# victorramirez952/tomography_3d_reconstructor

Measured on AMD Instinct MI355X. Metric: Mvoxels/s (SDF+MC) on 1024^3 ellipsoid stack; achieved HBM GB/s vs peak, higher is better.
Workload: dtype f64

## Files before the change

include/tomo_hip.h:

```cpp
#ifndef TOMO_HIP_H
#define TOMO_HIP_H

#include <stddef.h>
#include <stdint.h>

#ifdef __cplusplus
extern "C" {
#endif

#define TOMO_OK 0
#define TOMO_E_ARG (-1)
#define TOMO_E_LAUNCH (-2)
#define TOMO_E_SIZE (-3)
#define TOMO_E_WORKSPACE (-4)

int tomo_abi_version(void);
const char *tomo_error_string(int code);
int tomo_host_mc_cell(const float *h_v, double iso, int8_t *h_tris, int *h_uses_centre);
double tomo_host_mc_edge_offset(double va, double vb);
void tomo_host_mc_centre_offset(const double *h_v8, double *h_out3);

int tomo_host_checksum(const void *h_data, int64_t nbytes, int nthreads, uint64_t *h_out);
int tomo_host_checksum_impl(const void *h_data, int64_t nbytes, int nthreads, int impl, uint64_t *h_out);
int64_t tomo_host_checksum_chunk_bytes(void);
// ... 208 lines not shown
                        unsigned long long *vox_key, int64_t cap, void *stream);
int tomo_mc_eval_capped(const float *field, int Nz, int Ny, int Nx, int64_t pitch, int xorg, double iso,
                        const unsigned long long *vox_key, int64_t cap, const unsigned long long *na_dev,
                        uint32_t *vox_counts, uint8_t *vox_flags, void *stream);
int tomo_mc_emit(const float *field, int Nz, int Ny, int Nx, int64_t pitch, int xorg, double iso,
                 const unsigned long long *vox_key, int64_t na, const unsigned long long *seg_act,
                 const uint32_t *seg_aoff, const uint32_t *vox_voff, const uint32_t *vox_foff, const uint8_t *vox_flags,
                 int z_offset, unsigned long long *vkey, float *vpos, int32_t *faces, unsigned long long *totals,
                 void *stream);

int tomo_mc_first_touch(const float *field, int Nz, int Ny, int Nx, int64_t pitch, int xorg, double iso,
                        const unsigned long long *vox_key, int64_t na, const unsigned long long *seg_act,
                        const uint32_t *seg_aoff, const uint32_t *vox_voff, const uint8_t *vox_flags, int mode,
                        uint32_t *created, const uint32_t *base, int32_t *ft_rank, unsigned long long *totals, void *stream);

int tomo_mc3_list(int Nz, int Ny, int Nx, int xorg, const uint32_t *seg_cnt, const unsigned long long *seg_act,
                  uint32_t *seg_blk, uint32_t *seg_aoff, unsigned long long *vox_key, int64_t cap, unsigned long long *tot,
                  void *stream);
int tomo_mc3_eval(const float *field, int Nz, int Ny, int Nx, int64_t pitch, int xorg, double iso,
                  const unsigned long long *vox_key, int64_t cap, const unsigned long long *tot, int z_offset,
                  uint32_t *vox_loc, int32_t *vox_til, uint8_t *vox_flags, uint16_t *vox_used, float *vox_f3, float *vox_c3,
                  uint32_t *blk3, void *stream);
int64_t tomo_mc3_slice_table_words(int Nz, int Ny);
int64_t tomo_mc3_sort_segments(int Nz, int Ny);
int tomo_mc3_scan(int Nz, int Ny, int Nx, int xorg, const uint32_t *seg_aoff, const uint32_t *vox_loc, int64_t cap,
                  uint32_t *blk3, uint32_t *slice_tab, unsigned long long *tot, int64_t cap_v, int64_t cap_f, void *stream);
int tomo_mc3_vertices(int Nz, int Ny, int Nx, int xorg, const unsigned long long *vox_key, int64_t cap,
                      const unsigned long long *tot, const uint32_t *vox_loc, const uint8_t *vox_flags, const float *vox_f3,
                      const float *vox_c3, const uint32_t *blk3, const uint32_t *slice_tab, int z_offset, int shift,
                      const double *cum, int64_t ncum, const double *adj, int64_t nadj, float mm_y, float mm_x, float *vrec,
                      uint32_t *keys, uint32_t *idx, void *stream);
int64_t tomo_mc3_sort_workspace_bytes(int64_t cap_v, int64_t nseg);
int tomo_mc3_sort_rank_top(const float *vrec, uint32_t *keys, uint32_t *idx, int64_t cap_v, int Nz, int Ny, const uint32_t *slice_tab,
                           unsigned long long *tot, float *uniq, int32_t *table, void *workspace, int64_t workspace_bytes,
                           float z_top, void *stream);
int tomo_mc3_sort_rank_fused(const float *vrec, const uint32_t *keys, int64_t cap_v, int Nz, int Ny, uint32_t *slice_tab,
                             unsigned long long *tot, float *uniq, int32_t *table, float z_top, void *stream);
int tomo_mc3_faces(int Nz, int Ny, int Nx, int xorg, const unsigned long long *vox_key, int64_t cap, unsigned long long *tot,
                   const unsigned long long *seg_act, const uint32_t *seg_aoff, const uint32_t *vox_loc, const int32_t *vox_til,
                   const uint16_t *vox_used, const uint32_t *blk3, const int32_t *table, int64_t *faces, int64_t cap_f,
                   void *stream);
// ... 48 lines not shown
```

tomography_3d_reconstructor_amd/_lib.py:

```python
import ctypes
import os
import subprocess

_HERE = os.path.dirname(os.path.abspath(__file__))
SO_PATH = os.environ.get("TOMO_LIB") or os.path.join(_HERE, "libtomo_hip.so")
CSRC = os.path.join(_HERE, "csrc")

_c_i = ctypes.c_int
_c_i64 = ctypes.c_int64
_c_p = ctypes.c_void_p
_c_d = ctypes.c_double
_c_f = ctypes.c_float

SIGNATURES = {
    "tomo_abi_version": (_c_i, []),
    "tomo_error_string": (ctypes.c_char_p, [_c_i]),
    "tomo_host_mc_cell": (_c_i, [_c_p, _c_d, _c_p, _c_p]),
    "tomo_host_mc_edge_offset": (_c_d, [_c_d, _c_d]),
    "tomo_host_mc_centre_offset": (None, [_c_p, _c_p]),
    "tomo_host_checksum": (_c_i, [_c_p, _c_i64, _c_i, _c_p]),
    "tomo_host_checksum_impl": (_c_i, [_c_p, _c_i64, _c_i, _c_i, _c_p]),
    "tomo_host_checksum_chunk_bytes": (_c_i64, []),
    "tomo_host_checksum_part": (_c_i, [_c_p, _c_i64, _c_i64, _c_i, _c_i, _c_p]),
    "tomo_host_checksum_fold": (_c_i, [_c_p, _c_i64, _c_i64, _c_p]),
# ... 111 lines not shown
    "tomo_sign_rows": (_c_i64, [_c_i]),
    "tomo_sign_buffer_words": (_c_i64, [_c_i, _c_i, _c_i, _c_i]),
    "tomo_field_signs": (_c_i, [_c_p, _c_i, _c_i, _c_i, _c_i64, _c_i, _c_d, _c_i, _c_i, _c_p, _c_p, _c_p]),
    "tomo_mc_classify": (_c_i, [_c_p, _c_p, _c_i, _c_i, _c_i, _c_i, _c_p, _c_p, _c_p]),
    "tomo_mc_scan_segments": (_c_i, [_c_p, _c_i64, _c_p, _c_p, _c_p, _c_i64, _c_p]),
    "tomo_mc_scan_workspace_bytes": (_c_i64, [_c_i64]),
    "tomo_mc_scan": (_c_i, [_c_p, _c_i64, _c_p, _c_p, _c_p, _c_p, _c_i64, _c_p]),
    "tomo_mc_list": (_c_i, [_c_i, _c_i, _c_i, _c_i, _c_p, _c_p, _c_p, _c_p]),
    "tomo_mc_eval": (_c_i, [_c_p, _c_i, _c_i, _c_i, _c_i64, _c_i, _c_d, _c_p, _c_i64, _c_p, _c_p, _c_p]),
    "tomo_mc_list_capped": (_c_i, [_c_i, _c_i, _c_i, _c_i, _c_p, _c_p, _c_p, _c_i64, _c_p]),
    "tomo_mc_eval_capped": (_c_i, [_c_p, _c_i, _c_i, _c_i, _c_i64, _c_i, _c_d, _c_p, _c_i64, _c_p, _c_p, _c_p, _c_p]),
    "tomo_mc_emit": (_c_i, [_c_p, _c_i, _c_i, _c_i, _c_i64, _c_i, _c_d, _c_p, _c_i64, _c_p, _c_p, _c_p, _c_p, _c_p, _c_i, _c_p,
                            _c_p, _c_p, _c_p, _c_p]),
    "tomo_mc_first_touch": (_c_i, [_c_p, _c_i, _c_i, _c_i, _c_i64, _c_i, _c_d, _c_p, _c_i64, _c_p, _c_p, _c_p, _c_p, _c_i, _c_p,
                                   _c_p, _c_p, _c_p, _c_p]),
    "tomo_mc3_list": (_c_i, [_c_i, _c_i, _c_i, _c_i, _c_p, _c_p, _c_p, _c_p, _c_p, _c_i64, _c_p, _c_p]),
    "tomo_mc3_eval": (_c_i, [_c_p, _c_i, _c_i, _c_i, _c_i64, _c_i, _c_d, _c_p, _c_i64, _c_p, _c_i, _c_p, _c_p, _c_p, _c_p, _c_p,
                             _c_p, _c_p, _c_p]),
    "tomo_mc3_slice_table_words": (_c_i64, [_c_i, _c_i]),
    "tomo_mc3_sort_segments": (_c_i64, [_c_i, _c_i]),
    "tomo_mc3_scan": (_c_i, [_c_i, _c_i, _c_i, _c_i, _c_p, _c_p, _c_i64, _c_p, _c_p, _c_p, _c_i64, _c_i64, _c_p]),
    "tomo_mc3_vertices": (_c_i, [_c_i, _c_i, _c_i, _c_i, _c_p, _c_i64, _c_p, _c_p, _c_p, _c_p, _c_p, _c_p, _c_p, _c_i, _c_i,
                                 _c_p, _c_i64, _c_p, _c_i64, _c_f, _c_f, _c_p, _c_p, _c_p, _c_p]),
    "tomo_mc3_sort_workspace_bytes": (_c_i64, [_c_i64, _c_i64]),
    "tomo_mc3_sort_rank_top": (_c_i, [_c_p, _c_p, _c_p, _c_i64, _c_i, _c_i, _c_p, _c_p, _c_p, _c_p, _c_p, _c_i64, _c_f, _c_p]),
    "tomo_mc3_sort_rank_fused": (_c_i, [_c_p, _c_p, _c_i64, _c_i, _c_i, _c_p, _c_p, _c_p, _c_p, _c_f, _c_p]),
    "tomo_mc3_faces": (_c_i, [_c_i, _c_i, _c_i, _c_i, _c_p, _c_i64, _c_p, _c_p, _c_p, _c_p, _c_p, _c_p, _c_p, _c_p, _c_p, _c_i64, _c_p]),
    "tomo_vertex_finalize": (_c_i, [_c_p, _c_i64, _c_i, _c_p, _c_i64, _c_p, _c_i64, _c_f, _c_f, _c_p]),
    "tomo_mesh_unique_workspace_bytes": (_c_i64, [_c_i64]),
    "tomo_mesh_unique": (_c_i, [_c_p, _c_i64, _c_p, _c_p, _c_p, _c_p, _c_i64, _c_p]),
    "tomo_mesh_lookup": (_c_i, [_c_p, _c_i64, _c_p, _c_i64, _c_p, _c_p, _c_p]),
    "tomo_slab_top_rows": (_c_i, [_c_p, _c_p, _c_i64, _c_i64, _c_p, _c_p]),
    "tomo_slab_lookup_summary": (_c_i, [_c_p, _c_p, _c_i64, _c_p, _c_i64, _c_p, _c_i64, _c_i64, _c_p, _c_p, _c_p]),
    "tomo_mc3_faces_slab": (_c_i, [_c_i, _c_i, _c_i, _c_i, _c_p, _c_i64, _c_p, _c_p, _c_p, _c_p, _c_p, _c_p, _c_p, _c_p, _c_p, _c_i64,
                                   _c_p, _c_i, _c_i, _c_p, _c_i64, _c_i64, _c_p]),
    "tomo_mesh_volume_area": (_c_i, [_c_p, _c_p, _c_i64, _c_p, _c_p]),
# ... 60 lines not shown
```

tomography_3d_reconstructor_amd/csrc/mc.hip:

```cpp
#include <cstring>
#include <cstdlib>
#include "tomo_common.h"
#include <rocprim/rocprim.hpp>

#define MC_LUT_QUAL __device__ const
#define MC_FN __device__ static inline
#include "mc_cell.h"

#define SEG 256
#define KEY_XBITS 20
static_assert(KEY_XBITS + 2 == TOMO_KEY_ROW_SHIFT, "key layout shared with mesh.hip");

struct McGrid {
    int Nz, Ny, Nx;
    int64_t pitch;
    int xorg;
    int segs_per_row;
    double iso;
};

typedef float float4u __attribute__((ext_vector_type(4), aligned(4)));
typedef float float2u __attribute__((ext_vector_type(2), aligned(4)));
typedef float float3u __attribute__((ext_vector_type(3), aligned(4)));
typedef int int3u __attribute__((ext_vector_type(3), aligned(4)));
// ... 692 lines not shown
        return TOMO_E_ARG;
    if (na <= 0) return TOMO_OK;
    int64_t blocks = ceil_div64(na, 256);
    if (blocks > 0x7fffffff) return TOMO_E_SIZE;
    hipLaunchKernelGGL(mc_first_touch_kernel, dim3((unsigned)blocks), dim3(256), 0, (hipStream_t)stream, field, g,
                       (const u64 *)vox_key, na, (const u64 *)seg_act, seg_aoff, vox_voff, vox_flags, mode, created, base, ft_rank,
                       (u64 *)totals);
    return tomo_status();
}

#define MC3_BLK 256
#define MC3_LOC_A(l) ((l) & 1023u)
#define MC3_LOC_B(l) (((l) >> 10) & 1023u)
#define MC3_LOC_T(l) ((l) >> 20)

__global__ __launch_bounds__(256) void mc3_segsum_kernel(const u32 *__restrict__ seg_cnt, int64_t nseg, u32 *__restrict__ seg_blk,
                                                         int64_t nblk)
{
    const int lane = threadIdx.x & 63;
    const int64_t b = (int64_t)blockIdx.x * 4 + (threadIdx.x >> 6);
    if (b >= nblk) return;
    const int64_t i0 = b * MC3_BLK + lane * 4;
    u32 s = 0;
    if (i0 + 3 < nseg) {
        const uint4 v = *(const uint4 *)(seg_cnt + i0);
        s = v.x + v.y + v.z + v.w;
    } else {
        for (int k = 0; k < 4; k++) if (i0 + k < nseg) s += seg_cnt[i0 + k];
    }
    s = wave_sum(s);
    if (lane == 0) seg_blk[b] = s;
}

template <int K>
__device__ static inline void scan_small_inplace(u32 *__restrict__ a, int64_t stride, int64_t n, u64 *total_out, u32 *lds )
{
    const int lane = threadIdx.x & 63, w = threadIdx.x >> 6;
    u32 carry[K];
    u64 wide[K];
#pragma unroll
    for (int k = 0; k < K; k++) { carry[k] = 0; wide[k] = 0; }
    for (int64_t base = 0; base < n; base += 1024 * 8) {
        const int64_t i0 = base + (int64_t)threadIdx.x * 8;
        u32 v[K][8], s[K];
#pragma unroll
        for (int k = 0; k < K; k++) {
            u32 *p = a + k * stride + i0;
            if (i0 + 7 < n && ((uintptr_t)p & 15) == 0) {
                const uint4 lo = *(const uint4 *)p, hi = *(const uint4 *)(p + 4);
                v[k][0] = lo.x; v[k][1] = lo.y; v[k][2] = lo.z; v[k][3] = lo.w; v[k][4] = hi.x; v[k][5] = hi.y; v[k][6] = hi.z; v[k][7] = hi.w;
            } else {
#pragma unroll
                for (int j = 0; j < 8; j++) v[k][j] = i0 + j < n ? p[j] : 0u;
            }
            s[k] = 0;
#pragma unroll
            for (int j = 0; j < 8; j++) s[k] += v[k][j];
        }
        u32 inc[K];
#pragma unroll
        for (int k = 0; k < K; k++) {
            inc[k] = wave_inclusive_scan(s[k]);
            if (lane == 63) lds[k * 16 + w] = inc[k];
        }
        __syncthreads();
        if (w == 0) {
#pragma unroll
            for (int k = 0; k < K; k++) {
                const u32 t = lane < 16 ? lds[k * 16 + lane] : 0u;
                const u32 ti = wave_inclusive_scan(t);
                if (lane < 16) lds[k * 16 + lane] = ti - t;
                if (lane == 15) lds[K * 16 + k] = ti;
            }
        }
        __syncthreads();
#pragma unroll
        for (int k = 0; k < K; k++) {
            u32 ex = carry[k] + lds[k * 16 + w] + inc[k] - s[k];
            u32 *p = a + k * stride + i0;
            if (i0 + 7 < n && ((uintptr_t)p & 15) == 0) {
                uint4 lo, hi;
                lo.x = ex; ex += v[k][0]; lo.y = ex; ex += v[k][1]; lo.z = ex; ex += v[k][2]; lo.w = ex; ex += v[k][3];
                hi.x = ex; ex += v[k][4]; hi.y = ex; ex += v[k][5]; hi.z = ex; ex += v[k][6]; hi.w = ex;
                *(uint4 *)p = lo; *(uint4 *)(p + 4) = hi;
            } else {
#pragma unroll
                for (int j = 0; j < 8; j++) { if (i0 + j < n) p[j] = ex; ex += v[k][j]; }
            }
            carry[k] += lds[K * 16 + k];
            wide[k] += lds[K * 16 + k];
        }
        __syncthreads();
    }
#pragma unroll
    for (int k = 0; k < K; k++) total_out[k] = wide[k];
}

__global__ __launch_bounds__(1024) void mc3_scan_seg_kernel(u32 *__restrict__ seg_blk, int64_t nblk, u64 *__restrict__ tot)
{
    __shared__ u32 lds[17];
    u64 total;
    scan_small_inplace<1>(seg_blk, 0, nblk, &total, lds);
    if (threadIdx.x == 0) {
        tot[0] = total;
        tot[1] = tot[2] = tot[4] = tot[5] = tot[6] = tot[7] = 0ull;
        tot[3] = total > 0xffffffffull ? 1ull : 0ull;
    }
}

__global__ __launch_bounds__(MC3_BLK) void mc3_list_kernel(const McGrid g, const u32 *__restrict__ seg_cnt,
                                                           const u32 *__restrict__ seg_blk, const u64 *__restrict__ seg_act,
                                                           int64_t nseg, u32 *__restrict__ seg_aoff, u64 *__restrict__ vox_key,
                                                           u32 cap, u64 *__restrict__ tot)
{
    __shared__ u32 wsum[4];
    const int lane = threadIdx.x & 63, w = threadIdx.x >> 6;
    const int64_t seg = (int64_t)blockIdx.x * MC3_BLK + threadIdx.x;
    const u32 cnt = seg < nseg ? seg_cnt[seg] : 0u;
// ... 1 lines not shown
    if (lane == 63) wsum[w] = inc;
    __syncthreads();
    u32 o = seg_blk[blockIdx.x] + inc - cnt;
    for (int k = 0; k < w; k++) o += wsum[k];
    if (seg >= nseg) return;
    seg_aoff[seg] = o;
    if (seg == nseg - 1) seg_aoff[nseg] = o + cnt;
    if (cnt == 0) return;
    if ((u64)o + cnt > (u64)cap || tot[0] > (u64)cap) {
        if (o <= cap) atomicOr((unsigned long long *)&tot[3], 1ull);
        return;
    }
    seg_write_keys(g, seg, seg_act, o, vox_key);
}

TOMO_API int tomo_mc3_list(int Nz, int Ny, int Nx, int xorg, const uint32_t *seg_cnt, const unsigned long long *seg_act,
                           uint32_t *seg_blk, uint32_t *seg_aoff, unsigned long long *vox_key, int64_t cap,
                           unsigned long long *tot, void *stream)
{
    if (!seg_cnt || !seg_act || !seg_blk || !seg_aoff || !vox_key || !tot) return TOMO_E_ARG;
    McGrid g;
    if (const int rc = index_grid(g, Nz, Ny, Nx, xorg)) return rc;
    if (cap <= 0 || cap >= 0x1fffffffll) return TOMO_E_SIZE;
    const int64_t nseg = (int64_t)Nz * Ny * g.segs_per_row, nblk = ceil_div64(nseg, MC3_BLK);
    if (nblk > 0x7fffffff) return TOMO_E_SIZE;
    hipStream_t s = (hipStream_t)stream;
    hipLaunchKernelGGL(mc3_segsum_kernel, dim3((unsigned)ceil_div64(nblk, 4)), dim3(256), 0, s, seg_cnt, nseg, seg_blk, nblk);
    hipLaunchKernelGGL(mc3_scan_seg_kernel, dim3(1), dim3(1024), 0, s, seg_blk, nblk, (u64 *)tot);
    hipLaunchKernelGGL(mc3_list_kernel, dim3((unsigned)nblk), dim3(MC3_BLK), 0, s, g, seg_cnt, (const u32 *)seg_blk,
                       (const u64 *)seg_act, nseg, seg_aoff, (u64 *)vox_key, (u32)cap, (u64 *)tot);
    return tomo_status();
}

__global__ __launch_bounds__(MC3_BLK) void mc3_eval_kernel(const float *__restrict__ field, const McGrid g,
                                                           const u64 *__restrict__ vox_key, int64_t cap,
                                                           const u64 *__restrict__ tot, int z_offset,
                                                           u32 *__restrict__ vox_loc, int32_t *__restrict__ vox_til,
                                                           uint8_t *__restrict__ vox_flags, uint16_t *__restrict__ vox_used,
                                                           float *__restrict__ vox_f3, float *__restrict__ vox_c3,
                                                           u32 *__restrict__ blk3, int64_t nblk)
{
    __shared__ u32 wsum[4];
    const int lane = threadIdx.x & 63, w = threadIdx.x >> 6;
    const int64_t i = (int64_t)blockIdx.x * MC3_BLK + threadIdx.x;
    const u64 na = tot[0];
    const bool live = i < cap && (u64)i < na && na <= (u64)cap;
    u32 packed = 0;
    if (live) {
        Cell c;
        load_cell(field, g, vox_key[i], c);
        int ntri = 0;
        int32_t til = 0;
        u32 used = 0;
        if (c.cell_ok && c.index != 0 && c.index != 255) {
            const McTiling t = mc_cell_tiling(c.v, c.index);
// ... 15 lines not shown
            *(float3u *)(vox_c3 + 3 * i) = (float3u){(float)((double)Zg + oz), (float)((double)c.Y + oy), (float)((double)c.X + ox)};
        }
        vox_til[i] = til;
        vox_flags[i] = (uint8_t)c.flags;
        vox_used[i] = (uint16_t)used;
        packed = (u32)__popc(c.flags & 3) | ((u32)__popc(c.flags & 12) << 10) | ((u32)ntri << 20);
    }
    const u32 inc = wave_inclusive_scan(packed);
    if (lane == 63) wsum[w] = inc;
    __syncthreads();
    u32 ex = inc - packed;
    for (int k = 0; k < w; k++) ex += wsum[k];
    if (i < cap) vox_loc[i] = ex;
    if (threadIdx.x == MC3_BLK - 1) {
        const u32 sum = ex + packed;
        blk3[blockIdx.x] = MC3_LOC_A(sum);
        blk3[nblk + blockIdx.x] = MC3_LOC_B(sum);
        blk3[2 * nblk + blockIdx.x] = MC3_LOC_T(sum);
    }
}

__global__ __launch_bounds__(1024) void mc3_scan_kernel(const McGrid g, const u32 *__restrict__ seg_aoff,
                                                        const u32 *__restrict__ vox_loc, int64_t cap, u32 *__restrict__ blk3,
                                                        int64_t nblk, u32 *__restrict__ slice_tab, u64 *__restrict__ tot,
                                                        int64_t cap_v, int64_t cap_f)
{
    __shared__ u32 lds[3 * 16 + 3];
    u64 totals[3];
    scan_small_inplace<3>(blk3, nblk, nblk, totals, lds);
    const u64 na = tot[0];
    const u64 totA64 = totals[0], totB64 = totals[1], totT64 = totals[2];
    const u32 totA = (u32)totA64, totB = (u32)totB64;
    const int Nz = g.Nz;
    u32 *sliceA = slice_tab, *sliceB = slice_tab + (Nz + 1);
    const int64_t segs_per_slice = (int64_t)g.Ny * g.segs_per_row;
    const bool fits = na <= (u64)cap;
    for (int Z = threadIdx.x; Z <= Nz; Z += 1024) {
        u32 a = totA, b = totB;
        if (Z < Nz && fits) {
            const u64 s = seg_aoff[(int64_t)Z * segs_per_slice];
            if (s < na) {
                const u32 l = vox_loc[s];
                a = blk3[s >> 8] + MC3_LOC_A(l);
                b = blk3[nblk + (s >> 8)] + MC3_LOC_B(l);
            }
        }
        sliceA[Z] = a;
        sliceB[Z] = b;
    }
    u64 ov = 0;
    if (totA64 + totB64 > (u64)cap_v) ov |= 2ull;
    if (totT64 > (u64)cap_f) ov |= 4ull;
    if (!fits) ov |= 1ull;
    if (threadIdx.x == 0) {
        tot[1] = totA64 + totB64;
        tot[2] = totT64;
        if (ov) atomicOr((unsigned long long *)&tot[3], (unsigned long long)ov);
    }
}

__global__ __launch_bounds__(256) void mc3_bands_kernel(const McGrid g, const u32 *__restrict__ seg_aoff,
                                                        const u32 *__restrict__ vox_loc, const u32 *__restrict__ blk3,
                                                        int64_t nblk, u32 *__restrict__ slice_tab, const u64 *__restrict__ tot)
{
    const int Nz = g.Nz, NB = TOMO_SORT_NB(g.Ny);
    const int64_t nseg = (int64_t)(NB + 1) * Nz, i = (int64_t)blockIdx.x * blockDim.x + threadIdx.x;
    const u32 *sliceA = slice_tab, *sliceB = slice_tab + (Nz + 1);
    u32 *offsets = slice_tab + 2 * (Nz + 1), *merge3 = offsets + nseg + 1;
    const bool ov = tot[3] != 0;
// ... 169 lines not shown
                const int64_t j = row - k;
                dst[e] = row < k ? row + off_me : off_next + ((sm.ids_next && j < sm.cap_top) ? (int64_t)sm.ids_next[j] : 0);
            }
        } else {
            for (u32 e = threadIdx.x; e < n; e += MC3_BLK) dst[e] = (int64_t)sf[e];
        }
        __syncthreads();
    }
    if (degen) atomicAdd((unsigned long long *)&tot[5], (unsigned long long)degen);
    if (bad) atomicAdd((unsigned long long *)&tot[6], 1ull);
}

TOMO_API int tomo_mc3_eval(const float *field, int Nz, int Ny, int Nx, int64_t pitch, int xorg, double iso,
                           const unsigned long long *vox_key, int64_t cap, const unsigned long long *tot, int z_offset,
                           uint32_t *vox_loc, int32_t *vox_til, uint8_t *vox_flags, uint16_t *vox_used, float *vox_f3,
                           float *vox_c3, uint32_t *blk3, void *stream)
{
    McGrid g;
    if (const int rc = make_grid(g, field, Nz, Ny, Nx, pitch, xorg, iso)) return rc;
    if (!vox_key || !tot || !vox_loc || !vox_til || !vox_flags || !vox_used || !vox_f3 || !vox_c3 || !blk3 || cap <= 0) return TOMO_E_ARG;
    const int64_t nblk = ceil_div64(cap, MC3_BLK);
    if (nblk > 0x7fffffff) return TOMO_E_SIZE;
    hipLaunchKernelGGL(mc3_eval_kernel, dim3((unsigned)nblk), dim3(MC3_BLK), 0, (hipStream_t)stream, field, g, (const u64 *)vox_key,
                       cap, (const u64 *)tot, z_offset, vox_loc, vox_til, vox_flags, vox_used, vox_f3, vox_c3, blk3, nblk);
    return tomo_status();
}

TOMO_API int64_t tomo_mc3_sort_segments(int Nz, int Ny) { return (int64_t)(TOMO_SORT_NB(Ny) + 1) * Nz; }
TOMO_API int64_t tomo_mc3_slice_table_words(int Nz, int Ny) { return 2 * ((int64_t)Nz + 1) + tomo_mc3_sort_segments(Nz, Ny) + 1 + 3 + 8; }

TOMO_API int tomo_mc3_scan(int Nz, int Ny, int Nx, int xorg, const uint32_t *seg_aoff, const uint32_t *vox_loc, int64_t cap,
                           uint32_t *blk3, uint32_t *slice_tab, unsigned long long *tot, int64_t cap_v, int64_t cap_f,
                           void *stream)
{
    if (!seg_aoff || !vox_loc || !blk3 || !slice_tab || !tot || cap <= 0) return TOMO_E_ARG;
    McGrid g;
    if (const int rc = index_grid(g, Nz, Ny, Nx, xorg)) return rc;
    if (cap_v >= 0x7fffffffll || cap_f >= 0x7fffffffll) return TOMO_E_SIZE;
    hipLaunchKernelGGL(mc3_scan_kernel, dim3(1), dim3(1024), 0, (hipStream_t)stream, g, seg_aoff, vox_loc, cap, blk3,
                       ceil_div64(cap, MC3_BLK), slice_tab, (u64 *)tot, cap_v, cap_f);
    const int64_t nseg = tomo_mc3_sort_segments(Nz, Ny);
    if (nseg + 1 > 0x7fffffff) return TOMO_E_SIZE;
    hipLaunchKernelGGL(mc3_bands_kernel, dim3((unsigned)ceil_div64(nseg + 1, 256)), dim3(256), 0, (hipStream_t)stream, g, seg_aoff,
                       vox_loc, (const u32 *)blk3, ceil_div64(cap, MC3_BLK), slice_tab, (const u64 *)tot);
    return tomo_status();
}

TOMO_API int tomo_mc3_vertices(int Nz, int Ny, int Nx, int xorg, const unsigned long long *vox_key, int64_t cap,
                               const unsigned long long *tot, const uint32_t *vox_loc, const uint8_t *vox_flags,
                               const float *vox_f3, const float *vox_c3, const uint32_t *blk3, const uint32_t *slice_tab,
                               int z_offset, int shift, const double *cum, int64_t ncum, const double *adj, int64_t nadj,
                               float mm_y, float mm_x, float *vrec, uint32_t *keys, uint32_t *idx, void *stream)
{
    if (!vox_key || !tot || !vox_loc || !vox_flags || !vox_f3 || !vox_c3 || !blk3 || !slice_tab || !vrec || !keys || cap <= 0 ||
        (nadj > 0 && (!cum || !adj || ncum != nadj + 1)))
        return TOMO_E_ARG;
    McGrid g;
    if (const int rc = index_grid(g, Nz, Ny, Nx, xorg)) return rc;
    Mc3Final fin; fin.cum = cum; fin.adj = adj; fin.ncum = ncum; fin.nadj = nadj; fin.shift = shift; fin.mm_y = mm_y; fin.mm_x = mm_x;
// ... 41 lines not shown
```

tomography_3d_reconstructor_amd/pipeline.py:

```python
import math
import os
import threading
from dataclasses import dataclass

import numpy as np
import torch

from . import _lib


COUNTERS = dict.fromkeys(("na_hint_hit", "na_hint_miss", "mc3_hint_hit", "mc3_hint_miss", "mc3_sort_fused", "mc3_sort_library",
                          "mc3_exact", "mc3_general_unique", "mc3_degenerate", "components_label", "components_expand",
                          "components_filter", "slab_components_label", "slab_components_seam", "slab_components_merge",
                          "slab_components_expand", "slab_components_filter", "distance_transform", "distance_offset",
                          "components_measure", "components_zhist", "components_moments", "components_euler",
                          "components_cavities", "local_thickness", "opening_volume", "components_surface", "components_fill",
                          "components_cavity_owners", "component_thickness", "components_value", "components_levels", "component_caliper",
                          "geodesic_calls", "geodesic_sweeps", "component_geodesic", "zone_calls", "zone_sweeps", "zone_cuts",
                          "separate_components", "zone_contacts", "contact_launches"), 0)
NA_HINTS = os.environ.get("TOMO_NA_HINTS", "1") not in ("", "0")
_NA_HINT = {}
LIST_LIMIT = 2 ** 31
MESH_LIMIT = 2 ** 31
PACK_CLOSE_FUSED = os.environ.get("TOMO_PACK_CLOSE", "1") not in ("", "0")
# ... 2226 lines not shown
        self.nv = self.nf = self.na = 0
        self.deferred = False
        self._pending = None

    def classify(self):
        L, f, dev = _lib.lib(), self.field, self.field.data.device
        if f.signs is None or f.signs_level != 0.5:
            if f.sparse:
                raise _lib.TomoError("a sparse field holds floats only near the 0.5 surface")
            field_signs(f, 0.5)
        nseg = f.Nz * f.Ny * L.tomo_mc_segments_per_row(f.Nx, f.xorg)
        self.seg_act = torch.empty(nseg * 4, dtype=torch.int64, device=dev)
        self.seg_cnt = torch.empty(nseg, dtype=torch.int32, device=dev)
        _lib.check(L.tomo_mc_classify(_p(f.signs), _p(f.gcls), f.Nz, f.Ny, f.Nx, f.xorg, _p(self.seg_act), _p(self.seg_cnt), _stream()),
                   "tomo_mc_classify")
        self.seg_blk = torch.empty((nseg + 255) // 256, dtype=torch.int32, device=dev)
        self.seg_aoff = torch.empty(nseg + 1, dtype=torch.int32, device=dev)

    def build_list(self, cap):
        f, self.cap = self.field, cap
        self.vox_key = torch.empty(cap, dtype=torch.int64, device=f.data.device)
        _lib.check(_lib.lib().tomo_mc3_list(f.Nz, f.Ny, f.Nx, f.xorg, _p(self.seg_cnt), _p(self.seg_act), _p(self.seg_blk), _p(self.seg_aoff),
                                            _p(self.vox_key), cap, _p(self.tot), _stream()), "tomo_mc3_list")

    def eval_scan(self, cap_v, cap_f):
        L, f, cap, st, dev = _lib.lib(), self.field, self.cap, _stream(), self.field.data.device
        self.vox_loc = torch.empty(cap, dtype=torch.int32, device=dev)
        self.vox_til = torch.empty(cap, dtype=torch.int32, device=dev)
        self.vox_flags = torch.empty(cap, dtype=torch.uint8, device=dev)
        self.vox_used = torch.empty(cap, dtype=torch.int16, device=dev)
        self.vox_f3 = torch.empty(3 * cap, dtype=torch.float32, device=dev)
        self.vox_c3 = torch.empty(3 * cap, dtype=torch.float32, device=dev)
        self.blk3 = torch.empty(3 * ((cap + 255) // 256), dtype=torch.int32, device=dev)
        self.slice_tab = torch.empty(L.tomo_mc3_slice_table_words(f.Nz, f.Ny), dtype=torch.int32, device=dev)
        _lib.check(L.tomo_mc3_eval(_p(f.data), f.Nz, f.Ny, f.Nx, f.pitch, f.xorg, 0.5, _p(self.vox_key), cap, _p(self.tot), self.z_offset,
                                   _p(self.vox_loc), _p(self.vox_til), _p(self.vox_flags), _p(self.vox_used), _p(self.vox_f3),
                                   _p(self.vox_c3), _p(self.blk3), st), "tomo_mc3_eval")
        _lib.check(L.tomo_mc3_scan(f.Nz, f.Ny, f.Nx, f.xorg, _p(self.seg_aoff), _p(self.vox_loc), cap, _p(self.blk3), _p(self.slice_tab),
                                   _p(self.tot), cap_v, cap_f, st), "tomo_mc3_scan")

    def vertices_sort(self, cap_v):
        L, f, cap, tot, st, dev = _lib.lib(), self.field, self.cap, self.tot, _stream(), self.field.data.device
        cum_t, ncum, adj_t, nadj = self._depth
        self.cap_v = cap_v
        self.vrec = torch.empty((cap_v, 4), dtype=torch.float32, device=dev)
        keys = torch.empty(cap_v, dtype=torch.int32, device=dev)
        self.rows = torch.empty((cap_v, 3), dtype=torch.float32, device=dev)
        self.table = torch.empty(4 * cap, dtype=torch.int32, device=dev)
        fused = FUSED_SORT and not _MC3_LARGE.get(self.hint_key)
        idx = None if fused else torch.empty(cap_v, dtype=torch.int32, device=dev)
        _lib.check(L.tomo_mc3_vertices(f.Nz, f.Ny, f.Nx, f.xorg, _p(self.vox_key), cap, _p(tot), _p(self.vox_loc), _p(self.vox_flags),
                                       _p(self.vox_f3), _p(self.vox_c3), _p(self.blk3), _p(self.slice_tab), self.z_offset, 1, _p(cum_t), ncum,
                                       _p(adj_t), nadj, *self._mm, _p(self.vrec), _p(keys), _p(idx), st), "tomo_mc3_vertices")
        if fused:
# ... 428 lines not shown
```

Before: 707,800.

## Replace single-block scans of block sums with multi-block reduce-then-scan

```diff
diff --git a/include/tomo_hip.h b/include/tomo_hip.h
--- a/include/tomo_hip.h
+++ b/include/tomo_hip.h
@@ -246,17 +246,20 @@
                         const uint32_t *seg_aoff, const uint32_t *vox_voff, const uint8_t *vox_flags, int mode,
                         uint32_t *created, const uint32_t *base, int32_t *ft_rank, unsigned long long *totals, void *stream);
 
-int tomo_mc3_list(int Nz, int Ny, int Nx, int xorg, const uint32_t *seg_cnt, const unsigned long long *seg_act,
-                  uint32_t *seg_blk, uint32_t *seg_aoff, unsigned long long *vox_key, int64_t cap, unsigned long long *tot,
-                  void *stream);
+int64_t tomo_mc3_scan_range(void);
+int64_t tomo_mc3_scan_two_level(void);
+int tomo_mc3_build_list(int Nz, int Ny, int Nx, int xorg, const uint32_t *seg_cnt, const unsigned long long *seg_act,
+                        uint32_t *seg_sum, uint32_t *seg_blk, uint32_t *seg_aoff, unsigned long long *vox_key, int64_t cap,
+                        unsigned long long *tot, void *stream);
 int tomo_mc3_eval(const float *field, int Nz, int Ny, int Nx, int64_t pitch, int xorg, double iso,
                   const unsigned long long *vox_key, int64_t cap, const unsigned long long *tot, int z_offset,
                   uint32_t *vox_loc, int32_t *vox_til, uint8_t *vox_flags, uint16_t *vox_used, float *vox_f3, float *vox_c3,
-                  uint32_t *blk3, void *stream);
+                  uint32_t *sum3, void *stream);
 int64_t tomo_mc3_slice_table_words(int Nz, int Ny);
 int64_t tomo_mc3_sort_segments(int Nz, int Ny);
-int tomo_mc3_scan(int Nz, int Ny, int Nx, int xorg, const uint32_t *seg_aoff, const uint32_t *vox_loc, int64_t cap,
-                  uint32_t *blk3, uint32_t *slice_tab, unsigned long long *tot, int64_t cap_v, int64_t cap_f, void *stream);
+int tomo_mc3_scan_blocks(int Nz, int Ny, int Nx, int xorg, const uint32_t *seg_aoff, const uint32_t *vox_loc, int64_t cap,
+                         const uint32_t *sum3, uint32_t *blk3, uint32_t *slice_tab, unsigned long long *tot, int64_t cap_v,
+                         int64_t cap_f, void *stream);
 int tomo_mc3_vertices(int Nz, int Ny, int Nx, int xorg, const unsigned long long *vox_key, int64_t cap,
                       const unsigned long long *tot, const uint32_t *vox_loc, const uint8_t *vox_flags, const float *vox_f3,
                       const float *vox_c3, const uint32_t *blk3, const uint32_t *slice_tab, int z_offset, int shift,
diff --git a/tomography_3d_reconstructor_amd/_lib.py b/tomography_3d_reconstructor_amd/_lib.py
--- a/tomography_3d_reconstructor_amd/_lib.py
+++ b/tomography_3d_reconstructor_amd/_lib.py
@@ -149,12 +149,14 @@
                             _c_p, _c_p, _c_p, _c_p]),
     "tomo_mc_first_touch": (_c_i, [_c_p, _c_i, _c_i, _c_i, _c_i64, _c_i, _c_d, _c_p, _c_i64, _c_p, _c_p, _c_p, _c_p, _c_i, _c_p,
                                    _c_p, _c_p, _c_p, _c_p]),
-    "tomo_mc3_list": (_c_i, [_c_i, _c_i, _c_i, _c_i, _c_p, _c_p, _c_p, _c_p, _c_p, _c_i64, _c_p, _c_p]),
+    "tomo_mc3_scan_range": (_c_i64, []),
+    "tomo_mc3_scan_two_level": (_c_i64, []),
+    "tomo_mc3_build_list": (_c_i, [_c_i, _c_i, _c_i, _c_i, _c_p, _c_p, _c_p, _c_p, _c_p, _c_p, _c_i64, _c_p, _c_p]),
     "tomo_mc3_eval": (_c_i, [_c_p, _c_i, _c_i, _c_i, _c_i64, _c_i, _c_d, _c_p, _c_i64, _c_p, _c_i, _c_p, _c_p, _c_p, _c_p, _c_p,
                              _c_p, _c_p, _c_p]),
     "tomo_mc3_slice_table_words": (_c_i64, [_c_i, _c_i]),
     "tomo_mc3_sort_segments": (_c_i64, [_c_i, _c_i]),
-    "tomo_mc3_scan": (_c_i, [_c_i, _c_i, _c_i, _c_i, _c_p, _c_p, _c_i64, _c_p, _c_p, _c_p, _c_i64, _c_i64, _c_p]),
+    "tomo_mc3_scan_blocks": (_c_i, [_c_i, _c_i, _c_i, _c_i, _c_p, _c_p, _c_i64, _c_p, _c_p, _c_p, _c_p, _c_i64, _c_i64, _c_p]),
     "tomo_mc3_vertices": (_c_i, [_c_i, _c_i, _c_i, _c_i, _c_p, _c_i64, _c_p, _c_p, _c_p, _c_p, _c_p, _c_p, _c_p, _c_i, _c_i,
                                  _c_p, _c_i64, _c_p, _c_i64, _c_f, _c_f, _c_p, _c_p, _c_p, _c_p]),
     "tomo_mc3_sort_workspace_bytes": (_c_i64, [_c_i64, _c_i64]),
diff --git a/tomography_3d_reconstructor_amd/csrc/mc.hip b/tomography_3d_reconstructor_amd/csrc/mc.hip
--- a/tomography_3d_reconstructor_amd/csrc/mc.hip
+++ b/tomography_3d_reconstructor_amd/csrc/mc.hip
@@ -730,7 +730,7 @@
 #define MC3_LOC_B(l) (((l) >> 10) & 1023u)
 #define MC3_LOC_T(l) ((l) >> 20)
 
-__global__ __launch_bounds__(256) void mc3_segsum_kernel(const u32 *__restrict__ seg_cnt, int64_t nseg, u32 *__restrict__ seg_blk,
+__global__ __launch_bounds__(256) void mc3_segsum_kernel(const u32 *__restrict__ seg_cnt, int64_t nseg, u32 *__restrict__ seg_sum,
                                                          int64_t nblk)
 {
     const int lane = threadIdx.x & 63;
@@ -745,79 +745,92 @@
         for (int k = 0; k < 4; k++) if (i0 + k < nseg) s += seg_cnt[i0 + k];
     }
     s = wave_sum(s);
-    if (lane == 0) seg_blk[b] = s;
-}
-
-template <int K>
-__device__ static inline void scan_small_inplace(u32 *__restrict__ a, int64_t stride, int64_t n, u64 *total_out, u32 *lds )
-{
+    if (lane == 0) seg_sum[b] = s;
+}
+
+#define MC3_SCAN_G 256
+#define MC3_SCAN_SEG_T 256
+#define MC3_SCAN_EVAL_T 256
+#define MC3_SCAN_TWO_LEVEL 32768
+static_assert(MC3_SCAN_G == MC3_BLK, "the second level is mc3_segsum_kernel over the block sums");
+
+template <int K, int T>
+__device__ static inline void scan_range(const u32 *__restrict__ raw, int64_t stride, int64_t n, const u32 *__restrict__ fsrc,
+                                         int64_t fstride, int64_t fn, u32 ex[K], u64 total[K], u64 *lds)
+{
+    static_assert(T % 64 == 0 && T >= MC3_SCAN_G && MC3_SCAN_G % 64 == 0, "one thread per owned entry, whole waves");
+    constexpr int W = T / 64;
     const int lane = threadIdx.x & 63, w = threadIdx.x >> 6;
-    u32 carry[K];
-    u64 wide[K];
-#pragma unroll
-    for (int k = 0; k < K; k++) { carry[k] = 0; wide[k] = 0; }
-    for (int64_t base = 0; base < n; base += 1024 * 8) {
-        const int64_t i0 = base + (int64_t)threadIdx.x * 8;
-        u32 v[K][8], s[K];
+    const int64_t first = (int64_t)blockIdx.x * MC3_SCAN_G, i = first + threadIdx.x;
+    const bool mine = threadIdx.x < MC3_SCAN_G && i < n;
+    u32 v[K];
+    u64 front[K];
+    const uint4 *q[K];
+    int64_t nq[K], nqmin = INT64_MAX;
+#pragma unroll
+    for (int k = 0; k < K; k++) {
+        v[k] = mine ? raw[k * stride + i] : 0u;
+        const u32 *a = fsrc + k * fstride;
+        int64_t head = (int64_t)((0 - ((uintptr_t)a >> 2)) & 3);
+        if (head > fn) head = fn;
+        front[k] = (int64_t)threadIdx.x < head ? a[threadIdx.x] : 0u;
+        q[k] = (const uint4 *)(a + head);
+        nq[k] = (fn - head) >> 2;
+        const int64_t tail = head + nq[k] * 4 + threadIdx.x;
+        if (tail < fn) front[k] += a[tail];
+        if (nq[k] < nqmin) nqmin = nq[k];
+    }
+    int64_t j = threadIdx.x;
+#pragma unroll 8
+    for (; j < nqmin; j += T) {
 #pragma unroll
         for (int k = 0; k < K; k++) {
-            u32 *p = a + k * stride + i0;
-            if (i0 + 7 < n && ((uintptr_t)p & 15) == 0) {
-                const uint4 lo = *(const uint4 *)p, hi = *(const uint4 *)(p + 4);
-                v[k][0] = lo.x; v[k][1] = lo.y; v[k][2] = lo.z; v[k][3] = lo.w; v[k][4] = hi.x; v[k][5] = hi.y; v[k][6] = hi.z; v[k][7] = hi.w;
-            } else {
-#pragma unroll
-                for (int j = 0; j < 8; j++) v[k][j] = i0 + j < n ? p[j] : 0u;
-            }
-            s[k] = 0;
-#pragma unroll
-            for (int j = 0; j < 8; j++) s[k] += v[k][j];
-        }
-        u32 inc[K];
-#pragma unroll
-        for (int k = 0; k < K; k++) {
-            inc[k] = wave_inclusive_scan(s[k]);
-            if (lane == 63) lds[k * 16 + w] = inc[k];
-        }
-        __syncthreads();
-        if (w == 0) {
-#pragma unroll
-            for (int k = 0; k < K; k++) {
-                const u32 t = lane < 16 ? lds[k * 16 + lane] : 0u;
-                const u32 ti = wave_inclusive_scan(t);
-                if (lane < 16) lds[k * 16 + lane] = ti - t;
-                if (lane == 15) lds[K * 16 + k] = ti;
-            }
-        }
-        __syncthreads();
-#pragma unroll
-        for (int k = 0; k < K; k++) {
-            u32 ex = carry[k] + lds[k * 16 + w] + inc[k] - s[k];
-            u32 *p = a + k * stride + i0;
-            if (i0 + 7 < n && ((uintptr_t)p & 15) == 0) {
-                uint4 lo, hi;
-                lo.x = ex; ex += v[k][0]; lo.y = ex; ex += v[k][1]; lo.z = ex; ex += v[k][2]; lo.w = ex; ex += v[k][3];
-                hi.x = ex; ex += v[k][4]; hi.y = ex; ex += v[k][5]; hi.z = ex; ex += v[k][6]; hi.w = ex;
-                *(uint4 *)p = lo; *(uint4 *)(p + 4) = hi;
-            } else {
-#pragma unroll
-                for (int j = 0; j < 8; j++) { if (i0 + j < n) p[j] = ex; ex += v[k][j]; }
-            }
-            carry[k] += lds[K * 16 + k];
-            wide[k] += lds[K * 16 + k];
-        }
-        __syncthreads();
-    }
-#pragma unroll
-    for (int k = 0; k < K; k++) total_out[k] = wide[k];
-}
-
-__global__ __launch_bounds__(1024) void mc3_scan_seg_kernel(u32 *__restrict__ seg_blk, int64_t nblk, u64 *__restrict__ tot)
-{
-    __shared__ u32 lds[17];
+            const uint4 t = q[k][j];
+            front[k] += (u64)t.x + t.y + t.z + t.w;
+        }
+    }
+#pragma unroll
+    for (int k = 0; k < K; k++) {
+        if (j < nq[k]) {
+            const uint4 t = q[k][j];
+            front[k] += (u64)t.x + t.y + t.z + t.w;
+        }
+    }
+#pragma unroll
+    for (int k = 0; k < K; k++) {
+        const u32 inc = wave_inclusive_scan(v[k]);
+        const u64 s = wave_sum64(front[k]);
+        if (lane == 63) { lds[(k * W + w) * 2] = s; lds[(k * W + w) * 2 + 1] = inc; }
+        ex[k] = inc - v[k];
+    }
+    __syncthreads();
+#pragma unroll
+    for (int k = 0; k < K; k++) {
+        u64 f = 0;
+        u32 before = 0, sum = 0;
+#pragma unroll 4
+        for (int j = 0; j < W; j++) {
+            f += lds[(k * W + j) * 2];
+            const u32 t = (u32)lds[(k * W + j) * 2 + 1];
+            if (j < w) before += t;
+            sum += t;
+        }
+        ex[k] += (u32)f + before;
+        total[k] = f + sum;
+    }
+}
+
+__global__ __launch_bounds__(MC3_SCAN_SEG_T) void mc3_scan_seg_kernel(const u32 *__restrict__ seg_sum, const u32 *__restrict__ sup,
+                                                                      u32 *__restrict__ seg_blk, int64_t nblk, u64 *__restrict__ tot)
+{
+    __shared__ u64 lds[2 * (MC3_SCAN_SEG_T / 64)];
+    u32 ex;
     u64 total;
-    scan_small_inplace<1>(seg_blk, 0, nblk, &total, lds);
-    if (threadIdx.x == 0) {
+    if (sup) scan_range<1, MC3_SCAN_SEG_T>(seg_sum, 0, nblk, sup, 0, (int64_t)blockIdx.x, &ex, &total, lds);
+    else scan_range<1, MC3_SCAN_SEG_T>(seg_sum, 0, nblk, seg_sum, 0, (int64_t)blockIdx.x * MC3_SCAN_G, &ex, &total, lds);
+    const int64_t i = (int64_t)blockIdx.x * MC3_SCAN_G + threadIdx.x;
+    if (threadIdx.x < MC3_SCAN_G && i < nblk) seg_blk[i] = ex;
+    if (blockIdx.x == gridDim.x - 1 && threadIdx.x == 0) {
         tot[0] = total;
         tot[1] = tot[2] = tot[4] = tot[5] = tot[6] = tot[7] = 0ull;
         tot[3] = total > 0xffffffffull ? 1ull : 0ull;
@@ -849,19 +862,30 @@
     seg_write_keys(g, seg, seg_act, o, vox_key);
 }
 
-TOMO_API int tomo_mc3_list(int Nz, int Ny, int Nx, int xorg, const uint32_t *seg_cnt, const unsigned long long *seg_act,
-                           uint32_t *seg_blk, uint32_t *seg_aoff, unsigned long long *vox_key, int64_t cap,
-                           unsigned long long *tot, void *stream)
-{
-    if (!seg_cnt || !seg_act || !seg_blk || !seg_aoff || !vox_key || !tot) return TOMO_E_ARG;
+TOMO_API int64_t tomo_mc3_scan_range(void) { return MC3_SCAN_G; }
+TOMO_API int64_t tomo_mc3_scan_two_level(void) { return MC3_SCAN_TWO_LEVEL; }
+
+TOMO_API int tomo_mc3_build_list(int Nz, int Ny, int Nx, int xorg, const uint32_t *seg_cnt, const unsigned long long *seg_act,
+                                 uint32_t *seg_sum, uint32_t *seg_blk, uint32_t *seg_aoff, unsigned long long *vox_key,
+                                 int64_t cap, unsigned long long *tot, void *stream)
+{
+    if (!seg_cnt || !seg_act || !seg_sum || !seg_blk || !seg_aoff || !vox_key || !tot || seg_sum == seg_blk) return TOMO_E_ARG;
     McGrid g;
     if (const int rc = index_grid(g, Nz, Ny, Nx, xorg)) return rc;
     if (cap <= 0 || cap >= 0x1fffffffll) return TOMO_E_SIZE;
     const int64_t nseg = (int64_t)Nz * Ny * g.segs_per_row, nblk = ceil_div64(nseg, MC3_BLK);
     if (nblk > 0x7fffffff) return TOMO_E_SIZE;
     hipStream_t s = (hipStream_t)stream;
-    hipLaunchKernelGGL(mc3_segsum_kernel, dim3((unsigned)ceil_div64(nblk, 4)), dim3(256), 0, s, seg_cnt, nseg, seg_blk, nblk);
-    hipLaunchKernelGGL(mc3_scan_seg_kernel, dim3(1), dim3(1024), 0, s, seg_blk, nblk, (u64 *)tot);
+    hipLaunchKernelGGL(mc3_segsum_kernel, dim3((unsigned)ceil_div64(nblk, 4)), dim3(256), 0, s, seg_cnt, nseg, seg_sum, nblk);
+    const u32 *sup = nullptr;
+    if (nblk > MC3_SCAN_TWO_LEVEL) {
+        const int64_t nsup = ceil_div64(nblk, MC3_SCAN_G);
+        hipLaunchKernelGGL(mc3_segsum_kernel, dim3((unsigned)ceil_div64(nsup, 4)), dim3(256), 0, s, (const u32 *)seg_sum, nblk,
+                           seg_sum + nblk, nsup);
+        sup = seg_sum + nblk;
+    }
+    hipLaunchKernelGGL(mc3_scan_seg_kernel, dim3((unsigned)ceil_div64(nblk, MC3_SCAN_G)), dim3(MC3_SCAN_SEG_T), 0, s,
+                       (const u32 *)seg_sum, sup, seg_blk, nblk, (u64 *)tot);
     hipLaunchKernelGGL(mc3_list_kernel, dim3((unsigned)nblk), dim3(MC3_BLK), 0, s, g, seg_cnt, (const u32 *)seg_blk,
                        (const u64 *)seg_act, nseg, seg_aoff, (u64 *)vox_key, (u32)cap, (u64 *)tot);
     return tomo_status();
@@ -873,7 +897,7 @@
                                                            u32 *__restrict__ vox_loc, int32_t *__restrict__ vox_til,
                                                            uint8_t *__restrict__ vox_flags, uint16_t *__restrict__ vox_used,
                                                            float *__restrict__ vox_f3, float *__restrict__ vox_c3,
-                                                           u32 *__restrict__ blk3, int64_t nblk)
+                                                           u32 *__restrict__ sum3, int64_t nblk)
 {
     __shared__ u32 wsum[4];
     const int lane = threadIdx.x & 63, w = threadIdx.x >> 6;
@@ -919,45 +943,86 @@
     if (i < cap) vox_loc[i] = ex;
     if (threadIdx.x == MC3_BLK - 1) {
         const u32 sum = ex + packed;
-        blk3[blockIdx.x] = MC3_LOC_A(sum);
-        blk3[nblk + blockIdx.x] = MC3_LOC_B(sum);
-        blk3[2 * nblk + blockIdx.x] = MC3_LOC_T(sum);
-    }
-}
-
-__global__ __launch_bounds__(1024) void mc3_scan_kernel(const McGrid g, const u32 *__restrict__ seg_aoff,
-                                                        const u32 *__restrict__ vox_loc, int64_t cap, u32 *__restrict__ blk3,
-                                                        int64_t nblk, u32 *__restrict__ slice_tab, u64 *__restrict__ tot,
-                                                        int64_t cap_v, int64_t cap_f)
-{
-    __shared__ u32 lds[3 * 16 + 3];
-    u64 totals[3];
-    scan_small_inplace<3>(blk3, nblk, nblk, totals, lds);
-    const u64 na = tot[0];
-    const u64 totA64 = totals[0], totB64 = totals[1], totT64 = totals[2];
-    const u32 totA = (u32)totA64, totB = (u32)totB64;
+        sum3[blockIdx.x] = MC3_LOC_A(sum);
+        sum3[nblk + blockIdx.x] = MC3_LOC_B(sum);
+        sum3[2 * nblk + blockIdx.x] = MC3_LOC_T(sum);
+    }
+}
+
+__global__ __launch_bounds__(MC3_SCAN_EVAL_T) void mc3_scan_kernel(const McGrid g, const u32 *__restrict__ seg_aoff,
+                                                              const u32 *__restrict__ vox_loc, int64_t cap,
+                                                              const u32 *__restrict__ sum3, u32 *__restrict__ blk3,
+                                                              int64_t nblk, u32 *__restrict__ slice_tab, u64 *__restrict__ tot,
+                                                              int64_t cap_v, int64_t cap_f)
+{
+    __shared__ u64 lds[3 * 2 * (MC3_SCAN_EVAL_T / 64)];
+    __shared__ u32 preA[MC3_SCAN_G], preB[MC3_SCAN_G];
+    const int64_t first = (int64_t)blockIdx.x * MC3_SCAN_G, i = first + threadIdx.x;
+    const bool last = blockIdx.x == gridDim.x - 1;
     const int Nz = g.Nz;
     u32 *sliceA = slice_tab, *sliceB = slice_tab + (Nz + 1);
     const int64_t segs_per_slice = (int64_t)g.Ny * g.segs_per_row;
+    const u64 na = tot[0];
     const bool fits = na <= (u64)cap;
-    for (int Z = threadIdx.x; Z <= Nz; Z += 1024) {
-        u32 a = totA, b = totB;
-        if (Z < Nz && fits) {
-            const u64 s = seg_aoff[(int64_t)Z * segs_per_slice];
-            if (s < na) {
-                const u32 l = vox_loc[s];
-                a = blk3[s >> 8] + MC3_LOC_A(l);
-                b = blk3[nblk + (s >> 8)] + MC3_LOC_B(l);
+    constexpr int SLICES = 8;
+    u64 s[SLICES];
+    u32 l[SLICES];
+#pragma unroll
+    for (int k = 0; k < SLICES; k++) {
+        const int Z = threadIdx.x + k * MC3_SCAN_EVAL_T;
+        s[k] = Z < Nz && fits ? (u64)seg_aoff[(int64_t)Z * segs_per_slice] : na;
+    }
+#pragma unroll
+    for (int k = 0; k < SLICES; k++) {
+        const int64_t b = (int64_t)(s[k] >> 8) - first;
+        l[k] = s[k] < na && b >= 0 && b < MC3_SCAN_G ? vox_loc[s[k]] : 0xffffffffu;
+    }
+    u32 ex[3];
+    u64 totals[3];
+    scan_range<3, MC3_SCAN_EVAL_T>(sum3, nblk, nblk, sum3, nblk, first, ex, totals, lds);
+    if (threadIdx.x < MC3_SCAN_G) {
+        preA[threadIdx.x] = ex[0];
+        preB[threadIdx.x] = ex[1];
+        if (i < nblk) {
+            blk3[i] = ex[0];
+            blk3[nblk + i] = ex[1];
+            blk3[2 * nblk + i] = ex[2];
+        }
+    }
+    __syncthreads();
+    const u64 totA64 = totals[0], totB64 = totals[1], totT64 = totals[2];
+#pragma unroll
+    for (int k = 0; k < SLICES; k++) {
+        const int Z = threadIdx.x + k * MC3_SCAN_EVAL_T;
+        if (Z > Nz) continue;
+        if (l[k] != 0xffffffffu) {
+            const int64_t b = (int64_t)(s[k] >> 8) - first;
+            sliceA[Z] = preA[b] + MC3_LOC_A(l[k]);
+            sliceB[Z] = preB[b] + MC3_LOC_B(l[k]);
+        } else if (s[k] >= na && last) {
+            sliceA[Z] = (u32)totA64;
+            sliceB[Z] = (u32)totB64;
+        }
+    }
+    for (int Z = threadIdx.x + SLICES * MC3_SCAN_EVAL_T; Z <= Nz; Z += MC3_SCAN_EVAL_T) {
+        const u64 sz = Z < Nz && fits ? (u64)seg_aoff[(int64_t)Z * segs_per_slice] : na;
+        if (sz < na) {
+            const int64_t b = (int64_t)(sz >> 8) - first;
+            if (b >= 0 && b < MC3_SCAN_G) {
+                const u32 lz = vox_loc[sz];
+                sliceA[Z] = preA[b] + MC3_LOC_A(lz);
+                sliceB[Z] = preB[b] + MC3_LOC_B(lz);
             }
-        }
-        sliceA[Z] = a;
-        sliceB[Z] = b;
-    }
-    u64 ov = 0;
-    if (totA64 + totB64 > (u64)cap_v) ov |= 2ull;
-    if (totT64 > (u64)cap_f) ov |= 4ull;
-    if (!fits) ov |= 1ull;
-    if (threadIdx.x == 0) {
+        } else if (last) {
+            sliceA[Z] = (u32)totA64;
+            sliceB[Z] = (u32)totB64;
+        }
+    }
+    if (last && threadIdx.x == 0) {
+        u64 ov = 0;
+        if (totA64 + totB64 > (u64)cap_v) ov |= 2ull;
+        if (totT64 > (u64)cap_f) ov |= 4ull;
+        if (!fits) ov |= 1ull;
         tot[1] = totA64 + totB64;
         tot[2] = totT64;
         if (ov) atomicOr((unsigned long long *)&tot[3], (unsigned long long)ov);
@@ -1157,35 +1222,37 @@
 TOMO_API int tomo_mc3_eval(const float *field, int Nz, int Ny, int Nx, int64_t pitch, int xorg, double iso,
                            const unsigned long long *vox_key, int64_t cap, const unsigned long long *tot, int z_offset,
                            uint32_t *vox_loc, int32_t *vox_til, uint8_t *vox_flags, uint16_t *vox_used, float *vox_f3,
-                           float *vox_c3, uint32_t *blk3, void *stream)
+                           float *vox_c3, uint32_t *sum3, void *stream)
 {
     McGrid g;
     if (const int rc = make_grid(g, field, Nz, Ny, Nx, pitch, xorg, iso)) return rc;
-    if (!vox_key || !tot || !vox_loc || !vox_til || !vox_flags || !vox_used || !vox_f3 || !vox_c3 || !blk3 || cap <= 0) return TOMO_E_ARG;
+    if (!vox_key || !tot || !vox_loc || !vox_til || !vox_flags || !vox_used || !vox_f3 || !vox_c3 || !sum3 || cap <= 0) return TOMO_E_ARG;
     const int64_t nblk = ceil_div64(cap, MC3_BLK);
     if (nblk > 0x7fffffff) return TOMO_E_SIZE;
     hipLaunchKernelGGL(mc3_eval_kernel, dim3((unsigned)nblk), dim3(MC3_BLK), 0, (hipStream_t)stream, field, g, (const u64 *)vox_key,
-                       cap, (const u64 *)tot, z_offset, vox_loc, vox_til, vox_flags, vox_used, vox_f3, vox_c3, blk3, nblk);
+                       cap, (const u64 *)tot, z_offset, vox_loc, vox_til, vox_flags, vox_used, vox_f3, vox_c3, sum3, nblk);
     return tomo_status();
 }
 
 TOMO_API int64_t tomo_mc3_sort_segments(int Nz, int Ny) { return (int64_t)(TOMO_SORT_NB(Ny) + 1) * Nz; }
 TOMO_API int64_t tomo_mc3_slice_table_words(int Nz, int Ny) { return 2 * ((int64_t)Nz + 1) + tomo_mc3_sort_segments(Nz, Ny) + 1 + 3 + 8; }
 
-TOMO_API int tomo_mc3_scan(int Nz, int Ny, int Nx, int xorg, const uint32_t *seg_aoff, const uint32_t *vox_loc, int64_t cap,
-                           uint32_t *blk3, uint32_t *slice_tab, unsigned long long *tot, int64_t cap_v, int64_t cap_f,
-                           void *stream)
-{
-    if (!seg_aoff || !vox_loc || !blk3 || !slice_tab || !tot || cap <= 0) return TOMO_E_ARG;
+TOMO_API int tomo_mc3_scan_blocks(int Nz, int Ny, int Nx, int xorg, const uint32_t *seg_aoff, const uint32_t *vox_loc, int64_t cap,
+                                  const uint32_t *sum3, uint32_t *blk3, uint32_t *slice_tab, unsigned long long *tot, int64_t cap_v,
+                                  int64_t cap_f, void *stream)
+{
+    if (!seg_aoff || !vox_loc || !sum3 || !blk3 || sum3 == blk3 || !slice_tab || !tot || cap <= 0) return TOMO_E_ARG;
     McGrid g;
     if (const int rc = index_grid(g, Nz, Ny, Nx, xorg)) return rc;
     if (cap_v >= 0x7fffffffll || cap_f >= 0x7fffffffll) return TOMO_E_SIZE;
-    hipLaunchKernelGGL(mc3_scan_kernel, dim3(1), dim3(1024), 0, (hipStream_t)stream, g, seg_aoff, vox_loc, cap, blk3,
-                       ceil_div64(cap, MC3_BLK), slice_tab, (u64 *)tot, cap_v, cap_f);
+    const int64_t nblk = ceil_div64(cap, MC3_BLK);
+    if (nblk > 0x7fffffff) return TOMO_E_SIZE;
+    hipLaunchKernelGGL(mc3_scan_kernel, dim3((unsigned)ceil_div64(nblk, MC3_SCAN_G)), dim3(MC3_SCAN_EVAL_T), 0, (hipStream_t)stream, g,
+                       seg_aoff, vox_loc, cap, sum3, blk3, nblk, slice_tab, (u64 *)tot, cap_v, cap_f);
     const int64_t nseg = tomo_mc3_sort_segments(Nz, Ny);
     if (nseg + 1 > 0x7fffffff) return TOMO_E_SIZE;
     hipLaunchKernelGGL(mc3_bands_kernel, dim3((unsigned)ceil_div64(nseg + 1, 256)), dim3(256), 0, (hipStream_t)stream, g, seg_aoff,
-                       vox_loc, (const u32 *)blk3, ceil_div64(cap, MC3_BLK), slice_tab, (const u64 *)tot);
+                       vox_loc, (const u32 *)blk3, nblk, slice_tab, (const u64 *)tot);
     return tomo_status();
 }
 
diff --git a/tomography_3d_reconstructor_amd/pipeline.py b/tomography_3d_reconstructor_amd/pipeline.py
--- a/tomography_3d_reconstructor_amd/pipeline.py
+++ b/tomography_3d_reconstructor_amd/pipeline.py
@@ -2264,14 +2264,17 @@
         self.seg_cnt = torch.empty(nseg, dtype=torch.int32, device=dev)
         _lib.check(L.tomo_mc_classify(_p(f.signs), _p(f.gcls), f.Nz, f.Ny, f.Nx, f.xorg, _p(self.seg_act), _p(self.seg_cnt), _stream()),
                    "tomo_mc_classify")
-        self.seg_blk = torch.empty((nseg + 255) // 256, dtype=torch.int32, device=dev)
+        nb = (nseg + 255) // 256
+        self.seg_sum = torch.empty(nb + -(-nb // L.tomo_mc3_scan_range()), dtype=torch.int32, device=dev)
+        self.seg_blk = torch.empty(nb, dtype=torch.int32, device=dev)
         self.seg_aoff = torch.empty(nseg + 1, dtype=torch.int32, device=dev)
 
     def build_list(self, cap):
         f, self.cap = self.field, cap
         self.vox_key = torch.empty(cap, dtype=torch.int64, device=f.data.device)
-        _lib.check(_lib.lib().tomo_mc3_list(f.Nz, f.Ny, f.Nx, f.xorg, _p(self.seg_cnt), _p(self.seg_act), _p(self.seg_blk), _p(self.seg_aoff),
-                                            _p(self.vox_key), cap, _p(self.tot), _stream()), "tomo_mc3_list")
+        _lib.check(_lib.lib().tomo_mc3_build_list(f.Nz, f.Ny, f.Nx, f.xorg, _p(self.seg_cnt), _p(self.seg_act), _p(self.seg_sum),
+                                                  _p(self.seg_blk), _p(self.seg_aoff), _p(self.vox_key), cap, _p(self.tot), _stream()),
+                   "tomo_mc3_build_list")
 
     def eval_scan(self, cap_v, cap_f):
         L, f, cap, st, dev = _lib.lib(), self.field, self.cap, _stream(), self.field.data.device
@@ -2281,13 +2284,14 @@
         self.vox_used = torch.empty(cap, dtype=torch.int16, device=dev)
         self.vox_f3 = torch.empty(3 * cap, dtype=torch.float32, device=dev)
         self.vox_c3 = torch.empty(3 * cap, dtype=torch.float32, device=dev)
+        self.sum3 = torch.empty(3 * ((cap + 255) // 256), dtype=torch.int32, device=dev)
         self.blk3 = torch.empty(3 * ((cap + 255) // 256), dtype=torch.int32, device=dev)
         self.slice_tab = torch.empty(L.tomo_mc3_slice_table_words(f.Nz, f.Ny), dtype=torch.int32, device=dev)
         _lib.check(L.tomo_mc3_eval(_p(f.data), f.Nz, f.Ny, f.Nx, f.pitch, f.xorg, 0.5, _p(self.vox_key), cap, _p(self.tot), self.z_offset,
                                    _p(self.vox_loc), _p(self.vox_til), _p(self.vox_flags), _p(self.vox_used), _p(self.vox_f3),
-                                   _p(self.vox_c3), _p(self.blk3), st), "tomo_mc3_eval")
-        _lib.check(L.tomo_mc3_scan(f.Nz, f.Ny, f.Nx, f.xorg, _p(self.seg_aoff), _p(self.vox_loc), cap, _p(self.blk3), _p(self.slice_tab),
-                                   _p(self.tot), cap_v, cap_f, st), "tomo_mc3_scan")
+                                   _p(self.vox_c3), _p(self.sum3), st), "tomo_mc3_eval")
+        _lib.check(L.tomo_mc3_scan_blocks(f.Nz, f.Ny, f.Nx, f.xorg, _p(self.seg_aoff), _p(self.vox_loc), cap, _p(self.sum3), _p(self.blk3),
+                                          _p(self.slice_tab), _p(self.tot), cap_v, cap_f, st), "tomo_mc3_scan_blocks")
 
     def vertices_sort(self, cap_v):
         L, f, cap, tot, st, dev = _lib.lib(), self.field, self.cap, self.tot, _stream(), self.field.data.device
```

New measurement: 701,800. No clear change (-0.9%).
